# JinPLu/VeloxSeg

Measured on AMD Instinct MI355X. Metric: training patches/s on 128^3 2-mod volumes (fwd+loss+bwd+allreduce+AdamW), higher is better.
Workload: dtype f32

## Files before the change

include/veloxseg_hip.h:

```cpp
#ifndef VELOXSEG_HIP_H
#define VELOXSEG_HIP_H

#ifdef __cplusplus
extern "C" {
#endif

#define VX_ABI_VERSION 1

int vx_abi_version(void);
const char* vx_last_error(void);

int vx_conv3d_fwd(const float* x, const float* x2, int C1, const float* w, const float* bias, float* y,
                  int B, int Cin, int Di, int Hi, int Wi, int Cout, int K, int S, int P, int G, int ps, void* stream);
int vx_conv3d_bwd_data(const float* dy, const float* w, const float* bias_like, float* dx, float* dx2, int C1,
                       int B, int Cin, int Di, int Hi, int Wi, int Cout, int K, int S, int P, int G, int ps,
                       int accumulate, void* stream);
int vx_conv3d_bwd_weight(const float* x, const float* x2, int C1, const float* dy, float* dw, float* db,
                         int B, int Cin, int Di, int Hi, int Wi, int Cout, int K, int S, int P, int G, int ps, void* stream);

int vx_conv3d_bwd_weight_tiled(const float* x, const float* x2, int C1, const float* dy, float* dw, float* db,
                               int B, int Cin, int Di, int Hi, int Wi, int Cout, int K, int S, int P, int G, int ps, void* stream);
int vx_down_wgrad_ws_floats(int B, int Cin, int Di, int Hi, int Wi, int Cout);
int vx_down_wgrad_mfma(const float* x, const float* dy, float* dw, float* db, float* ws, long ws_floats,
                       int B, int Cin, int Di, int Hi, int Wi, int Cout, void* stream);
// ... 33 lines not shown
int vx_pw_conv_set_v4(int on);
int vx_pw_conv_bwd_data(const float* dy, const float* w, float* dx, float* dx2, int C1,
                        int B, int Cin, int Cout, long V, int accumulate, void* stream);
int vx_pw_conv_bwd_weight(const float* x, const float* x2, int C1, const float* dy, float* dw, float* db,
                          int B, int Cin, int Cout, long V, void* stream);
int vx_pw_conv_fwd_h(const void* x, const float* w, const float* bias, float* y, int B, int Cin, int Cout, long V, int x_h16, void* stream);
int vx_pw_conv_bwd_weight_h(const void* x, const float* dy, float* dw, float* db, int B, int Cin, int Cout, long V, int x_h16, void* stream);

int vx_pw_conv_mfma(const float* src, const float* src2, int S1, const float* w, int transpose_w, const float* bias,
                    float* dst, float* dst2, int D1, int B, int Mch, int Kch, int Cin_of_w, long V, int accumulate, void* stream);
int vx_pw_conv_bwd_fused(const float* dy, const float* w, const float* x, const float* x2, int C1, float* dx, float* dx2, float* dw, float* db,
                         int B, int Cin, int Cout, long V, int accumulate, void* stream);
int vx_pw_conv_bwd_fused_big(const float* dy, const float* w, const float* x, const float* x2, int C1, float* dx, float* dx2, float* dw, float* db,
                             int B, int Cin, int Cout, long V, int accumulate, void* stream);
int vx_pw_conv_gelu_fwd(const float* x, const float* w, const float* bias, float* a, float* h, int B, int Cin, int Cout, long V, int mfma,
                        const void* seed_ptr, unsigned long long dstream, float p, void* stream);
int vx_pw_conv_gelu_bwd_data(const float* dy, const float* w, const float* a, float* da, int B, int Cin, int Cout, long V, int mfma,
                             const void* seed_ptr, unsigned long long dstream, float p, void* stream);
int vx_pw_conv_res_fwd(const float* x, const float* w, const float* bias, const float* res, float* out, int B, int Cin, int Cout, long V, int mfma,
                       float alpha, const void* seed_ptr, unsigned long long dstream, float p, void* stream);
int vx_pw_mfma_set_wide(int on);

int vx_mlp_supported(int C, int R, long V);
int vx_mlp_bwd_nparts(int B, int C, long V);
int vx_mlp_fwd(const float* x, int norm, const double* part, int nparts, float* stats, const float* gamma, const float* beta,
               const float* w1, const float* b1, const float* w2, const float* b2, float* out, int B, int C, int R, long V, float eps,
               const void* seed_ptr, unsigned long long site1, float p1, unsigned long long site2, float p2, void* stream);
int vx_mlp_bwd(const float* x, int norm, const float* stats, const float* gamma, const float* beta, const float* w1, const float* b1,
               const float* w2, const float* dout, float* dx, float* part_out, float* dgamma, float* dbeta, float* dw1, float* db1,
               float* dw2, float* db2, int B, int C, int R, long V, float eps, const void* seed_ptr, unsigned long long site1, float p1,
               unsigned long long site2, float p2, void* stream);
int vx_jlc_ntiles(int B, int C, int G, int D, int H, int W);
int vx_jlc_nchunks(long BC, long V);
int vx_jlc_conv_fwd(const float* x, const float* w1, const float* w3, const float* w5, const float* b1, const float* b3, const float* b5,
                    float* y1, float* y3, float* y5, double* part, int B, int C, int G, int D, int H, int W, void* stream);
int vx_jlc_mid_fwd(const float* x, const float* y1, const float* y3, const float* y5, const double* part_y, int nty, float* stats_y, float* o,
                   double* part_o, long BC, long V, float eps, void* stream);
int vx_jlc_mid_bwd(const float* dout, const float* dn, const float* part_dn, int npd, const float* o, const float* stats_o, const float* y1,
                   const float* y3, const float* y5, const float* stats_y, float* d_o, float* part_t, long BC, long V, void* stream);
int vx_jlc_gk(const float* d_o, const float* y1, const float* y3, const float* y5, const float* stats_y, const float* part_t, float* g1, float* g3,
              float* g5, long BC, long V, void* stream);
int vx_jlc_conv_bwd(const float* g1, const float* g3, const float* g5, const float* w1, const float* w3, const float* w5, const float* d_o,
                    float* dx, int B, int C, int G, int D, int H, int W, void* stream);
int vx_jlc_mid_fwd_h(const float* x, const void* y1, const void* y3, const void* y5, const double* part_y, int nty, float* stats_y, void* o,
                     double* part_o, long BC, long V, float eps, int h16, void* stream);
int vx_jlc_mid_bwd_h(const float* dout, const void* dn, const float* part_dn, int npd, const void* o, const float* stats_o, const void* y1,
                     const void* y3, const void* y5, const float* stats_y, void* d_o, float* part_t, long BC, long V, int h16, void* stream);
int vx_jlc_gk_h(const void* d_o, const void* y1, const void* y3, const void* y5, const float* stats_y, const float* part_t, void* g1, void* g3,
                void* g5, long BC, long V, int h16, void* stream);
int vx_mlp_fwd_h(const void* x, int norm, const double* part, int nparts, float* stats, const float* gamma, const float* beta,
                 const float* w1, const float* b1, const float* w2, const float* b2, float* out, int B, int C, int R, long V, float eps,
                 const void* seed_ptr, unsigned long long site1, float p1, unsigned long long site2, float p2, int h16, void* stream);
int vx_mlp_bwd_h(const void* x, int norm, const float* stats, const float* gamma, const float* beta, const float* w1, const float* b1,
                 const float* w2, const float* dout, void* dx, float* part_out, float* dgamma, float* dbeta, float* dw1, float* db1,
                 float* dw2, float* db2, int B, int C, int R, long V, float eps, const void* seed_ptr, unsigned long long site1, float p1,
                 unsigned long long site2, float p2, int h16, void* stream);

int vx_jlc_tz_ok(int C, int G, int D, int H, int W);
int vx_jlc_tz_ntiles(int C, int G, int D, int H, int W);
int vx_jlc_tz_img_floats(int C, int G);
int vx_jlc_tz_set_pieces(int ns);
int vx_jlc_tz_set_min_voxels(long v);
int vx_jlc_tz_pieces(void);
int vx_jlc_tz_set_debug(int mask);
int vx_jlc_tz_prep(const float* w1, const float* w3, const float* w5, float* img, int C, int G, void* stream);
int vx_jlc_tz_fwd(const float* x, const float* img, const float* b1, const float* b3, const float* b5, float* y1, float* y3, float* y5, double* part,
                  int B, int C, int G, int D, int H, int W, void* stream);
int vx_jlc_tz_bwd(const float* g1, const float* g3, const float* g5, const float* img, const float* w1, const float* d_o, float* dx,
                  int B, int C, int G, int D, int H, int W, void* stream);
int vx_jlc_cl_ok(int C, int G, int D, int H, int W);
int vx_jlc_cl_ntiles(int C, int G, int D, int H, int W);
int vx_jlc_cl_img_floats(int C, int G);
int vx_jlc_cl_set_enabled(int on);
int vx_jlc_cl_prep(const float* w1, const float* w3, const float* w5, float* img, int C, int G, void* stream);
int vx_jlc_cl_fwd(const float* x, const float* img, const float* b1, const float* b3, const float* b5, float* y1, float* y3, float* y5, double* part,
                  int B, int C, int G, int D, int H, int W, void* stream);
int vx_jlc_cl_bwd(const float* g1, const float* g3, const float* g5, const float* img, const float* d_o, float* dx, int B, int C, int G, int D, int H, int W,
                  void* stream);
int vx_jlc_wgrad_tz_ok(int C, int G, int D, int H, int W);
int vx_jlc_wgrad_tz_set_min_voxels(long v);
int vx_jlc_wgrad_tz_set_blocks(int n);
int vx_jlc_wgrad_tz_set_spec(int on);
int vx_jlc_wgrad_tz_set_f16(int on);
int vx_jlc_wgrad_tz(const float* x, const float* g1, const float* g3, const float* g5, float* dw1, float* dw3, float* dw5, int B, int C, int G, int D, int H, int W,
                    void* stream);
int vx_jlc_tz_img_floats_ns(int C, int G, int pieces);
int vx_jlc_tz_prep_ns(const float* w1, const float* w3, const float* w5, float* img, int C, int G, int pieces, void* stream);
int vx_jlc_tz_fwd_ns(const float* x, const float* img, const float* b1, const float* b3, const float* b5, float* y1, float* y3, float* y5, double* part,
                     int B, int C, int G, int D, int H, int W, int pieces, void* stream);
int vx_jlc_tz_bwd_ns(const float* g1, const float* g3, const float* g5, const float* img, const float* w1, const float* d_o, float* dx,
                     int B, int C, int G, int D, int H, int W, int pieces, void* stream);
int vx_jlc_wgrad_tz_ns(const float* x, const float* g1, const float* g3, const float* g5, float* dw1, float* dw3, float* dw5, int B, int C, int G, int D, int H, int W,
                       int pieces, void* stream);
int vx_jlc_tz_fwd_h(const float* x, const float* img, const float* b1, const float* b3, const float* b5, void* y1, void* y3, void* y5, double* part,
// ... 246 lines not shown
```

veloxseg_amd/csrc/_vxops.cpp:

```cpp
#include <torch/extension.h>
#include <torch/csrc/autograd/custom_function.h>
#include <torch/custom_class.h>
#include <torch/library.h>
#include <c10/hip/HIPStream.h>
#include <ATen/hip/impl/HIPStreamMasqueradingAsCUDA.h>
#include <ATen/hip/impl/HIPGuardImplMasqueradingAsCUDA.h>
#include <hip/hip_runtime_api.h>
#include <algorithm>
#include <map>
#include <unordered_map>
#include <tuple>
#include <functional>
#include <type_traits>
#include <memory>
#include <vector>
#include <map>
#include <tuple>
#include "../../include/veloxseg_hip.h"

using at::Tensor;
typedef c10::optional<Tensor> OptT;

namespace {

// ... 990 lines not shown
            out = axpy_fwd_impl(st->r, o, z, 1.0, p, site, sp(rs), s_);
        }
        return {out, st};
    }

static Tensor jlc_bwd_f(std::shared_ptr<JLCState> st, const Tensor& dout_in, bool need_x, int64_t stream) {
        void* s_ = sp(stream);
        if (st->blk) {
            JLCFusedState& f = st->f;
            Tensor dout = contig(dout_in);
            const int B = f.B, C = f.C, G = f.G, D = f.D, H = f.H, W = f.W, R = f.R;
            const long V = (long)D * H * W, BC = (long)B * C, n1 = BC * V;
            const int npd = f.tile ? vx_inmlp_tiles(V) : vx_mlp_bwd_nparts(B, C, V);
            auto iopt = f.h16 ? f.x.options().dtype(at::kBFloat16) : f.x.options();
            const long esz = f.h16 ? 2 : 4;
            const int h16 = f.h16 ? 1 : 0;
            Tensor dn = at::empty(f.x.sizes(), iopt), part_dn = at::empty({BC, (long)npd, 2}, f.x.options());
            if (f.tile) {
                Tensor sc_n = at::empty_like(f.x), sc_dz = at::empty_like(f.x), sc_h = at::empty({B, R, D, H, W}, f.x.options()), sc_da = at::empty({B, R, D, H, W}, f.x.options());
                VX(vx_inmlp_bwd, fp(f.o), fp(f.stats_o), fp(f.l1w), fp(f.l1b), fp(f.l2w), fp(dout), mp(dn), mp(part_dn), mp(sc_n), mp(sc_h), mp(sc_da), mp(sc_dz), B, C, R, V,
                                 f.rs, (unsigned long long)f.site, (float)f.p, s_);
                float *dw1 = grad_ptr(f.l1w), *db1 = grad_ptr(f.l1b), *dw2 = grad_ptr(f.l2w), *db2 = grad_ptr(f.l2b);
                wgrad_submit(s_, f.x.device().index(), [=](void* s) {
                    const void* ptrs[8] = {fp(sc_h), fp(sc_dz), dw2, db2, fp(sc_n), fp(sc_da), dw1, db1};
                    const long dims[8] = {R, C, V, B, C, R, V, B};
                    VX(vx_pw_wgrad_group, ptrs, dims, 2, nullptr, nullptr, 0, s);
                });
            } else
            VX(vx_mlp_bwd_h, (const void*)f.o.data_ptr(), 0, fp(f.stats_o), nullptr, nullptr, fp(f.l1w), fp(f.l1b), fp(f.l2w), fp(dout), dn.data_ptr(), mp(part_dn), nullptr, nullptr,
                           grad_ptr(f.l1w), grad_ptr(f.l1b), grad_ptr(f.l2w), grad_ptr(f.l2b), B, C, R, V, (float)F.in_eps, f.rs, 0ull, 0.0f,
                           (unsigned long long)f.site, (float)f.p, h16, s_);
            const char* yp = (const char*)f.y.data_ptr();
            const void *y1 = yp, *y3 = yp + esz * n1, *y5 = yp + 2 * esz * n1;
            Tensor d_o = at::empty(f.x.sizes(), iopt), part_t = at::empty({3, BC, (long)f.nch, 2}, f.x.options());
            VX(vx_jlc_mid_bwd_h, fp(dout), (const void*)dn.data_ptr(), fp(part_dn), npd, (const void*)f.o.data_ptr(), fp(f.stats_o), y1, y3, y5, fp(f.stats_y), d_o.data_ptr(), mp(part_t), BC, V, h16, s_);
            Tensor g = at::empty({3, B, C, D, H, W}, iopt);
            char* gp = (char*)g.data_ptr();
            void *g1 = gp, *g3 = gp + esz * n1, *g5 = gp + 2 * esz * n1;
            VX(vx_jlc_gk_h, (const void*)d_o.data_ptr(), y1, y3, y5, fp(f.stats_y), fp(part_t), g1, g3, g5, BC, V, h16, s_);
            Tensor dx;
            if (need_x) {
                dx = f.h16 ? at::empty_like(f.x) : dn;
                if (f.img.defined() && f.img_cl) VX(vx_jlc_cl_bwd, (const float*)g1, (const float*)g3, (const float*)g5, fp(f.img), fp(d_o), mp(dx), B, C, G, D, H, W, s_);
                else if (f.img.defined()) VX(vx_jlc_tz_bwd_h, (const void*)g1, (const void*)g3, (const void*)g5, fp(f.img), fp(f.w1), (const void*)d_o.data_ptr(), mp(dx), B, C, G, D, H, W, f.tz_pieces, h16, s_);
                else
                VX(vx_jlc_conv_bwd, (const float*)g1, (const float*)g3, (const float*)g5, fp(f.w1), fp(f.w3), fp(f.w5), fp(d_o), mp(dx), B, C, G, D, H, W, s_);
            }
            grad_ptr(f.b1); grad_ptr(f.b3); grad_ptr(f.b5);
            const int Cg = C / G;
            {
                Tensor xk = f.x, gk = g;
                float* dw1 = f.w1.requires_grad() ? grad_ptr(f.w1) : nullptr;
                float* dw3 = f.w3.requires_grad() ? grad_ptr(f.w3) : nullptr;
                float* dw5 = f.w5.requires_grad() ? grad_ptr(f.w5) : nullptr;
                const bool g1fast = F.use_gconv1 && (Cg == 4 || Cg == 8 || Cg == 16) && V % 4 == 0;
                const bool tzok = F.jlc_wg_tz && dw1 && dw3 && dw5 && vx_jlc_wgrad_tz_ok(C, G, D, H, W);
                const bool wga = F.jlc_wg_tz && dw1 && dw3 && dw5 && vx_jlc_wgrad_gather_ok(C, G, D, H, W) == 1 && (!tzok || V <= 64);
                const bool wtz = !wga && tzok;
                const int wg_pieces = f.tz_pieces ? f.tz_pieces : vx_jlc_tz_pieces();
                wgrad_submit(s_, f.x.device().index(), [=](void* s) {
                    if (h16) {
                        const char* gh = (const char*)gk.data_ptr();
                        TORCH_CHECK(wtz, "veloxseg_amd.jlc: the 16-bit g_k of the bf16 storage mode need the matrix-pipe weight-gradient kernel");
                        VX(vx_jlc_wgrad_tz_h, fp(xk), (const void*)gh, (const void*)(gh + 2 * n1), (const void*)(gh + 4 * n1), dw1, dw3, dw5, B, C, G, D, H, W, wg_pieces, 1, s);
                        return;
                    }
                    const float* gq = gk.data_ptr<float>();
                    if (wga) {
                        VX(vx_jlc_wgrad_gather, fp(xk), gq, gq + n1, gq + 2 * n1, dw1, dw3, dw5, B, C, G, D, H, W, s);
                        return;
                    }
                    if (wtz) {
// ... 642 lines not shown
```

veloxseg_amd/csrc/jlc.hip:

```cpp
#include "vx_common.h"
#include "../../include/veloxseg_hip.h"

struct VxJlc {
    const float *x, *w1, *w3, *w5, *b1, *b3, *b5;
    const float *g1, *g3, *g5, *res;
    float *y1, *y3, *y5, *dx;
    double* part;
    int B, C, G, D, H, W;
    int TD, TH, TWq, nTd, nTh, nTw, cic, nthr;
    int parts, nsp;
};

template <int K>
__device__ __forceinline__ void vx_jlc_stage(const float* __restrict__ src, float* __restrict__ xs, const VxJlc& p, int b, int c_first, int ncc,
                                             int d0, int h0, int w0, int HD, int HH, int HWp) {
    constexpr int P = K / 2;
    const int tid = threadIdx.x, nthr = p.nthr;
    int hw = tid % HWp, t1 = tid / HWp;
    int hh = t1 % HH, t2 = t1 / HH;
    int hd = t2 % HD, cil = t2 / HD;
    int r = nthr;
    const int st_hw = r % HWp; r /= HWp;
    const int st_hh = r % HH; r /= HH;
    const int st_hd = r % HD; r /= HD;
// ... 361 lines not shown
            st[2 * k] = mean; st[2 * k + 1] = rstd;
            if (blockIdx.x == 0) { p.stats_y_out[((long)k * p.BC + bc) * 2] = mean; p.stats_y_out[((long)k * p.BC + bc) * 2 + 1] = rstd; }
        }
    }
    __syncthreads();
    const float m1 = st[0], r1 = st[1], m3 = st[2], r3 = st[3], m5 = st[4], r5 = st[5];
    const long base = bc * p.V, c0 = (long)blockIdx.x * p.chunk;
    const long c1 = c0 + p.chunk < p.V ? c0 + p.chunk : p.V;
    float s = 0.0f, q = 0.0f;
    for (long i = c0 + 4 * tid; i < c1; i += 1024) {
        const float4 xv = vx_ld4(p.x, base + i), a = vx_ld4(y1, base + i), b3 = vx_ld4(y3, base + i), c5 = vx_ld4(y5, base + i);
        float4 o;
        o.x = xv.x + vx_gelu_fast((a.x - m1) * r1) + vx_gelu_fast((b3.x - m3) * r3) + vx_gelu_fast((c5.x - m5) * r5);
        o.y = xv.y + vx_gelu_fast((a.y - m1) * r1) + vx_gelu_fast((b3.y - m3) * r3) + vx_gelu_fast((c5.y - m5) * r5);
        o.z = xv.z + vx_gelu_fast((a.z - m1) * r1) + vx_gelu_fast((b3.z - m3) * r3) + vx_gelu_fast((c5.z - m5) * r5);
        o.w = xv.w + vx_gelu_fast((a.w - m1) * r1) + vx_gelu_fast((b3.w - m3) * r3) + vx_gelu_fast((c5.w - m5) * r5);
        o.x = vx_round_as<TI>(o.x); o.y = vx_round_as<TI>(o.y); o.z = vx_round_as<TI>(o.z); o.w = vx_round_as<TI>(o.w);
        vx_st4(out_o, base + i, o);
        s += (o.x + o.y) + (o.z + o.w);
        q = fmaf(o.x, o.x, q); q = fmaf(o.y, o.y, q); q = fmaf(o.z, o.z, q); q = fmaf(o.w, o.w, q);
    }
    s = vx_wave_sum(s);
    q = vx_wave_sum(q);
    if ((tid & 63) == 0) { redd[2 * (tid >> 6)] = (double)s; redd[2 * (tid >> 6) + 1] = (double)q; }
    __syncthreads();
    if (tid == 0) {
        double* dst = p.part_o + (bc * p.nch + blockIdx.x) * 2;
        dst[0] = (redd[0] + redd[2]) + (redd[4] + redd[6]);
        dst[1] = (redd[1] + redd[3]) + (redd[5] + redd[7]);
    }
}

template <typename TI>
__global__ void __launch_bounds__(256) vx_jlc_mid_bwd_k(VxJlcMid p) {
    const TI* __restrict__ y1 = (const TI*)p.y1; const TI* __restrict__ y3 = (const TI*)p.y3; const TI* __restrict__ y5 = (const TI*)p.y5;
    const TI* __restrict__ o_ = (const TI*)p.o; const TI* __restrict__ dn_ = (const TI*)p.dn;
    TI* __restrict__ out_do = (TI*)p.out_do;
    __shared__ float mm[2];
    __shared__ float redf[4][6];
    const long bc = blockIdx.y;
    const int tid = threadIdx.x;
    if (tid < 64) {
        float s, q;
        vx_fold_f(p.part_dn + bc * p.npd * 2, p.npd, s, q);
        if (tid == 0) { mm[0] = s / (float)p.V; mm[1] = q / (float)p.V; }
    }
    __syncthreads();
    const float dm1 = mm[0], dm2 = mm[1];
    const float mo = p.stats_o[2 * bc], ro = p.stats_o[2 * bc + 1];
    float mk[3], rk[3];
#pragma unroll
    for (int k = 0; k < 3; ++k) { mk[k] = p.stats_y[((long)k * p.BC + bc) * 2]; rk[k] = p.stats_y[((long)k * p.BC + bc) * 2 + 1]; }
    const long base = bc * p.V, c0 = (long)blockIdx.x * p.chunk;
    const long c1 = c0 + p.chunk < p.V ? c0 + p.chunk : p.V;
    float acc[6] = {0.f, 0.f, 0.f, 0.f, 0.f, 0.f};
    for (long i = c0 + 4 * tid; i < c1; i += 1024) {
        const float4 go = vx_ld4(p.dout, base + i), dn = vx_ld4(dn_, base + i), ov = vx_ld4(o_, base + i);
        const float4 a = vx_ld4(y1, base + i), b3 = vx_ld4(y3, base + i), c5 = vx_ld4(y5, base + i);
        const float gov[4] = {go.x, go.y, go.z, go.w}, dnv[4] = {dn.x, dn.y, dn.z, dn.w}, oo[4] = {ov.x, ov.y, ov.z, ov.w};
        const float yv[3][4] = {{a.x, a.y, a.z, a.w}, {b3.x, b3.y, b3.z, b3.w}, {c5.x, c5.y, c5.z, c5.w}};
        float dv[4];
#pragma unroll
        for (int u = 0; u < 4; ++u) {
            const float nh = (oo[u] - mo) * ro;
            dv[u] = vx_round_as<TI>(gov[u] + ro * (dnv[u] - dm1 - nh * dm2));
#pragma unroll
            for (int k = 0; k < 3; ++k) {
                const float yh = (yv[k][u] - mk[k]) * rk[k];
                const float t = dv[u] * vx_gelu_grad_fast(yh);
                acc[2 * k] += t;
                acc[2 * k + 1] = fmaf(t, yh, acc[2 * k + 1]);
            }
        }
        vx_st4(out_do, base + i, make_float4(dv[0], dv[1], dv[2], dv[3]));
    }
#pragma unroll
    for (int e = 0; e < 6; ++e) {
        const float t = vx_wave_sum(acc[e]);
        if ((tid & 63) == 0) redf[tid >> 6][e] = t;
    }
    __syncthreads();
    if (tid < 6) {
        const int k = tid >> 1;
        p.part_t[(((long)k * p.BC + bc) * p.nch + blockIdx.x) * 2 + (tid & 1)] = (redf[0][tid] + redf[1][tid]) + (redf[2][tid] + redf[3][tid]);
    }
}

template <typename TI>
__global__ void __launch_bounds__(256) vx_jlc_gk_k(VxJlcMid p) {
    const TI* __restrict__ y1 = (const TI*)p.y1; const TI* __restrict__ y3 = (const TI*)p.y3; const TI* __restrict__ y5 = (const TI*)p.y5;
    const TI* __restrict__ d_o = (const TI*)p.d_o;
    TI* __restrict__ g1 = (TI*)p.g1; TI* __restrict__ g3 = (TI*)p.g3; TI* __restrict__ g5 = (TI*)p.g5;
    __shared__ float mm[6];
    const long bc = blockIdx.y;
    const int tid = threadIdx.x;
    if (tid < 192) {
        const int k = tid >> 6;
        float s, q;
        vx_fold_f(p.part_t_in + ((long)k * p.BC + bc) * p.nch * 2, p.nch, s, q);
        if ((tid & 63) == 0) { mm[2 * k] = s / (float)p.V; mm[2 * k + 1] = q / (float)p.V; }
    }
    __syncthreads();
    float mk[3], rk[3], t1[3], t2[3];
#pragma unroll
    for (int k = 0; k < 3; ++k) {
        mk[k] = p.stats_y[((long)k * p.BC + bc) * 2]; rk[k] = p.stats_y[((long)k * p.BC + bc) * 2 + 1];
        t1[k] = mm[2 * k]; t2[k] = mm[2 * k + 1];
    }
    const long base = bc * p.V, c0 = (long)blockIdx.x * p.chunk;
    const long c1 = c0 + p.chunk < p.V ? c0 + p.chunk : p.V;
    for (long i = c0 + 4 * tid; i < c1; i += 1024) {
        const float4 dv = vx_ld4(d_o, base + i);
        const float4 a = vx_ld4(y1, base + i), b3 = vx_ld4(y3, base + i), c5 = vx_ld4(y5, base + i);
        const float d4[4] = {dv.x, dv.y, dv.z, dv.w};
        const float yv[3][4] = {{a.x, a.y, a.z, a.w}, {b3.x, b3.y, b3.z, b3.w}, {c5.x, c5.y, c5.z, c5.w}};
        float gk[3][4];
#pragma unroll
        for (int k = 0; k < 3; ++k)
#pragma unroll
            for (int u = 0; u < 4; ++u) {
                const float yh = (yv[k][u] - mk[k]) * rk[k];
                const float t = d4[u] * vx_gelu_grad_fast(yh);
                gk[k][u] = rk[k] * (t - t1[k] - yh * t2[k]);
            }
        vx_st4(g1, base + i, make_float4(gk[0][0], gk[0][1], gk[0][2], gk[0][3]));
        vx_st4(g3, base + i, make_float4(gk[1][0], gk[1][1], gk[1][2], gk[1][3]));
        vx_st4(g5, base + i, make_float4(gk[2][0], gk[2][1], gk[2][2], gk[2][3]));
    }
}

static int vx_jlc_geom(VxJlc& p, int B, int C, int G, int D, int H, int W, int K, int& COT, size_t& shm) {
    VX_REQUIRE(B > 0 && C > 0 && G > 0 && C % G == 0 && D > 0 && H > 0 && W > 0, "vx_jlc: bad shape");
    const int Cg = C / G;
    VX_REQUIRE(Cg % 4 == 0, "vx_jlc: group width must be a multiple of 4 (got %d)", Cg);
    p.B = B; p.C = C; p.G = G; p.D = D; p.H = H; p.W = W;
    p.TWq = vx_cdiv(W, 4) < 8 ? vx_cdiv(W, 4) : 8;
    p.TH = H < 8 ? H : 8;
    int td = 256 / (p.TWq * p.TH);
    if (td > D) td = D;
    if (td > 8) td = 8;
    if (td < 1) td = 1;
    p.TD = td;
    auto nblk = [&]() { return (long)vx_cdiv(D, p.TD) * vx_cdiv(H, p.TH) * vx_cdiv(W, p.TWq * 4) * (C / COT) * 4; };
    COT = 4;
    while (p.TD > 1 && nblk() < 128 && (p.TD / 2) * p.TWq * p.TH >= 64) p.TD /= 2;
    p.nTd = vx_cdiv(D, p.TD); p.nTh = vx_cdiv(H, p.TH); p.nTw = vx_cdiv(W, p.TWq * 4);
    p.nsp = (p.TD * p.TH * p.TWq + 63) / 64 * 64;
    if (p.nsp > 256) p.nsp = 256;
    const int plane = (p.TD + K - 1) * (p.TH + K - 1) * (p.TWq * 4 + 4);
    const int taps = K == 5 ? 153 : 125;
    int cic = Cg < 4 ? Cg : 4;
    auto lds = [&](int c) { return (size_t)c * (plane + taps * COT) * sizeof(float); };
    while (cic > 1 && lds(cic) > 64 * 1024) cic >>= 1;
    p.parts = 1;
    if (nblk() < 512) {
        if (cic % 4 == 0 && p.nsp * 4 <= 512 && nblk() < 384) p.parts = 4;
        else if (cic % 2 == 0 && p.nsp * 2 <= 512) p.parts = 2;
    }
    p.nthr = p.nsp * p.parts;
    p.cic = cic;
// ... 12 lines not shown

extern "C" int vx_jlc_conv_fwd(const float* x, const float* w1, const float* w3, const float* w5, const float* b1, const float* b3, const float* b5,
                               float* y1, float* y3, float* y5, double* part, int B, int C, int G, int D, int H, int W, void* stream) {
    VX_REQUIRE(x && w1 && w3 && w5 && y1 && y3 && y5 && part, "vx_jlc_conv_fwd: null pointer");
    VxJlc p = {};
    int COT; size_t shm;
    if (int rc = vx_jlc_geom(p, B, C, G, D, H, W, 5, COT, shm)) return rc;
    p.x = x; p.w1 = w1; p.w3 = w3; p.w5 = w5; p.b1 = b1; p.b3 = b3; p.b5 = b5; p.y1 = y1; p.y3 = y3; p.y5 = y5; p.part = part;
    dim3 grid(p.nTd * p.nTh * p.nTw, C / COT, B);
    hipStream_t st = (hipStream_t)stream;
    if (COT == 4) vx_jlc_conv_fwd_k<4><<<grid, dim3(p.nthr), shm, st>>>(p);
    else if (COT == 2) vx_jlc_conv_fwd_k<2><<<grid, dim3(p.nthr), shm, st>>>(p);
    else vx_jlc_conv_fwd_k<1><<<grid, dim3(p.nthr), shm, st>>>(p);
    VX_LAUNCH_CHECK("vx_jlc_conv_fwd");
    return 0;
}

extern "C" int vx_jlc_conv_bwd(const float* g1, const float* g3, const float* g5, const float* w1, const float* w3, const float* w5, const float* d_o,
                               float* dx, int B, int C, int G, int D, int H, int W, void* stream) {
    VX_REQUIRE(g1 && g3 && g5 && w1 && w3 && w5 && d_o && dx, "vx_jlc_conv_bwd: null pointer");
    VxJlc p = {};
    int COT; size_t shm;
    if (int rc = vx_jlc_geom(p, B, C, G, D, H, W, 5, COT, shm)) return rc;
    p.g1 = g1; p.g3 = g3; p.g5 = g5; p.w1 = w1; p.w3 = w3; p.w5 = w5; p.res = d_o; p.dx = dx;
    dim3 grid(p.nTd * p.nTh * p.nTw, C / COT, B);
    hipStream_t st = (hipStream_t)stream;
    if (COT == 4) vx_jlc_conv_bwd_k<4><<<grid, dim3(p.nthr), shm, st>>>(p);
    else if (COT == 2) vx_jlc_conv_bwd_k<2><<<grid, dim3(p.nthr), shm, st>>>(p);
    else vx_jlc_conv_bwd_k<1><<<grid, dim3(p.nthr), shm, st>>>(p);
    VX_LAUNCH_CHECK("vx_jlc_conv_bwd");
    return 0;
}

static long vx_jlc_chunk(long BC, long V) {
    (void)BC;
    return V >= 16384 ? 4096 : 1024;
}
extern "C" int vx_jlc_nchunks(long BC, long V) { return vx_cdiv(V, vx_jlc_chunk(BC, V)); }

extern "C" int vx_jlc_mid_fwd_h(const float* x, const void* y1, const void* y3, const void* y5, const double* part_y, int nty, float* stats_y, void* o,
                                double* part_o, long BC, long V, float eps, int h16, void* stream) {
    VX_REQUIRE(x && y1 && y3 && y5 && part_y && stats_y && o && part_o && BC > 0 && V > 0 && V % 4 == 0, "vx_jlc_mid_fwd: bad args");
    VxJlcMid p = {};
    p.x = x; p.y1 = y1; p.y3 = y3; p.y5 = y5; p.part_y = part_y; p.nty = nty; p.stats_y_out = stats_y; p.out_o = o; p.part_o = part_o;
    p.BC = BC; p.V = V; p.eps = eps; p.chunk = vx_jlc_chunk(BC, V); p.nch = vx_cdiv(V, p.chunk);
    if (h16) vx_jlc_mid_fwd_k<vx_bf16><<<dim3(p.nch, (unsigned)BC), dim3(256), 0, (hipStream_t)stream>>>(p);
    else vx_jlc_mid_fwd_k<float><<<dim3(p.nch, (unsigned)BC), dim3(256), 0, (hipStream_t)stream>>>(p);
    VX_LAUNCH_CHECK("vx_jlc_mid_fwd");
    return 0;
}
extern "C" int vx_jlc_mid_fwd(const float* x, const float* y1, const float* y3, const float* y5, const double* part_y, int nty, float* stats_y, float* o,
                              double* part_o, long BC, long V, float eps, void* stream) {
    return vx_jlc_mid_fwd_h(x, y1, y3, y5, part_y, nty, stats_y, o, part_o, BC, V, eps, 0, stream);
}

extern "C" int vx_jlc_mid_bwd_h(const float* dout, const void* dn, const float* part_dn, int npd, const void* o, const float* stats_o, const void* y1,
                                const void* y3, const void* y5, const float* stats_y, void* d_o, float* part_t, long BC, long V, int h16, void* stream) {
    VX_REQUIRE(dout && dn && part_dn && o && stats_o && y1 && y3 && y5 && stats_y && d_o && part_t && BC > 0 && V > 0 && V % 4 == 0, "vx_jlc_mid_bwd: bad args");
    VxJlcMid p = {};
    p.dout = dout; p.dn = dn; p.part_dn = part_dn; p.npd = npd; p.o = o; p.stats_o = stats_o; p.y1 = y1; p.y3 = y3; p.y5 = y5; p.stats_y = stats_y;
    p.out_do = d_o; p.part_t = part_t; p.BC = BC; p.V = V; p.chunk = vx_jlc_chunk(BC, V); p.nch = vx_cdiv(V, p.chunk);
    if (h16) vx_jlc_mid_bwd_k<vx_bf16><<<dim3(p.nch, (unsigned)BC), dim3(256), 0, (hipStream_t)stream>>>(p);
    else vx_jlc_mid_bwd_k<float><<<dim3(p.nch, (unsigned)BC), dim3(256), 0, (hipStream_t)stream>>>(p);
    VX_LAUNCH_CHECK("vx_jlc_mid_bwd");
    return 0;
}
extern "C" int vx_jlc_mid_bwd(const float* dout, const float* dn, const float* part_dn, int npd, const float* o, const float* stats_o, const float* y1,
                              const float* y3, const float* y5, const float* stats_y, float* d_o, float* part_t, long BC, long V, void* stream) {
    return vx_jlc_mid_bwd_h(dout, dn, part_dn, npd, o, stats_o, y1, y3, y5, stats_y, d_o, part_t, BC, V, 0, stream);
}

extern "C" int vx_jlc_gk_h(const void* d_o, const void* y1, const void* y3, const void* y5, const float* stats_y, const float* part_t, void* g1, void* g3,
                           void* g5, long BC, long V, int h16, void* stream) {
    VX_REQUIRE(d_o && y1 && y3 && y5 && stats_y && part_t && g1 && g3 && g5 && BC > 0 && V > 0 && V % 4 == 0, "vx_jlc_gk: bad args");
    VxJlcMid p = {};
    p.d_o = d_o; p.y1 = y1; p.y3 = y3; p.y5 = y5; p.stats_y = stats_y; p.part_t_in = part_t; p.g1 = g1; p.g3 = g3; p.g5 = g5;
    p.BC = BC; p.V = V; p.chunk = vx_jlc_chunk(BC, V); p.nch = vx_cdiv(V, p.chunk);
    if (h16) vx_jlc_gk_k<vx_bf16><<<dim3(p.nch, (unsigned)BC), dim3(256), 0, (hipStream_t)stream>>>(p);
    else vx_jlc_gk_k<float><<<dim3(p.nch, (unsigned)BC), dim3(256), 0, (hipStream_t)stream>>>(p);
    VX_LAUNCH_CHECK("vx_jlc_gk");
    return 0;
}
extern "C" int vx_jlc_gk(const float* d_o, const float* y1, const float* y3, const float* y5, const float* stats_y, const float* part_t, float* g1, float* g3,
                         float* g5, long BC, long V, void* stream) {
    return vx_jlc_gk_h(d_o, y1, y3, y5, stats_y, part_t, g1, g3, g5, BC, V, 0, stream);
}
```

veloxseg_amd/csrc/jlc_mfma.hip:

```cpp
#include "vx_common.h"
#include <type_traits>
#include "../../include/veloxseg_hip.h"

typedef __bf16 tz_bf8 __attribute__((ext_vector_type(8)));
typedef float tz_f4 __attribute__((ext_vector_type(4)));

struct TzGeo {
    int HD, HH;
    int Sd, Sc, Sp;
    int nrows;
    unsigned mHH, mHD;
    int qd0, nq;
    unsigned mNQ;
};

struct VxTz {
    const void* src[3];
    const uint4* img;
    const float* esc;
    const float* bias[3];
    const void* res;
    const float* w1;
    void* out[3];
    double* part;
// ... 522 lines not shown
static unsigned tz_magic(int d) { return d <= 1 ? 0u : (unsigned)(((1ull << 32) + d - 1) / (unsigned long long)d); }

static int g_tz_pieces = 22;
static thread_local int t_tz_pieces = 0;
static inline int tz_pieces() { return t_tz_pieces ? t_tz_pieces : g_tz_pieces; }
namespace { struct TzPiecesScope { int prev; explicit TzPiecesScope(int ns) : prev(t_tz_pieces) { t_tz_pieces = ns; } ~TzPiecesScope() { t_tz_pieces = prev; } }; }
static inline bool tz_pieces_valid(int ns) { return (ns >= 1 && ns <= 3) || ns == 22; }
static thread_local int t_tz_h16 = 0;
namespace { struct TzH16Scope { int prev; explicit TzH16Scope(int h) : prev(t_tz_h16) { t_tz_h16 = h; } ~TzH16Scope() { t_tz_h16 = prev; } }; }
static int g_tz_dbg = 0;
extern "C" int vx_jlc_tz_set_debug(int mask) { g_tz_dbg = mask; return 0; }
extern "C" int vx_jlc_tz_set_pieces(int ns) { if (!((ns >= 1 && ns <= 3) || ns == 22)) return -1; g_tz_pieces = ns; return 0; }
static inline int tz_ns(int pieces) { return pieces == 22 ? 2 : pieces; }
extern "C" int vx_jlc_tz_pieces(void) { return g_tz_pieces; }

struct TzPlan { int CG, NT, MTW, nwaves; size_t shm; };

static void tz_geo(TzGeo& ge, const VxTz& p, int CG, int hw) {
    ge.HD = p.TD + 2 * hw; ge.HH = p.TH + 2 * hw;
    ge.Sd = ge.HH * p.RW;
    if (p.TWB >= 2) {
        const int iv = 4 * p.TWB;
        while (!((ge.Sd % iv) == 0 && ((ge.Sd / iv) & 1) && true)) ge.Sd += 4;
    }
    ge.Sc = ge.HD * ge.Sd;
    while ((ge.Sc & 127) != 64) ge.Sc += 4;
    ge.Sp = CG * ge.Sc;
    ge.nrows = CG * ge.HD * ge.HH;
    ge.mHH = tz_magic(ge.HH); ge.mHD = tz_magic(ge.HD);
    if (hw == 0) { ge.qd0 = 1; ge.nq = p.TWB; } else { ge.qd0 = 0; ge.nq = p.TWB + 2; }
    ge.mNQ = tz_magic(ge.nq);
}

static int tz_plan(VxTz& p, TzPlan& pl, int B, int C, int G, int D, int H, int W, int pieces) {
    const int NS = tz_ns(pieces);
    if (B <= 0 || C <= 0 || G <= 0 || C % G || D <= 0 || H <= 0 || W <= 0 || (W & 3)) return -1;
    const int CG = C / G;
    if (CG != 4 && CG != 8 && CG != 16) return -1;
    p.B = B; p.C = C; p.G = G; p.D = D; p.H = H; p.W = W;
    constexpr int tdm = 8, thm = 8;
    p.TWB = W / 4 < 8 ? W / 4 : 8;
    p.TH = H < thm ? H : thm;
    p.TD = D < tdm ? D : tdm;
    auto lds_bytes = [&](int td, int th, int twb) {
        VxTz q = p; TzGeo ge;
        q.TD = td; q.TH = th; q.TWB = twb; q.RW = 4 * twb + 4;
        tz_geo(ge, q, CG, 2);
        return (size_t)NS * ge.Sp * 2;
    };
    while (lds_bytes(p.TD, p.TH, p.TWB) > 150 * 1024) {
        if (p.TD > 1 && p.TD >= p.TH) p.TD = (p.TD + 1) / 2;
        else if (p.TH > 1) p.TH = (p.TH + 1) / 2;
        else return -1;
    }
    p.nTd = vx_cdiv(D, p.TD); p.nTh = vx_cdiv(H, p.TH); p.nTw = vx_cdiv(W / 4, p.TWB);
    p.RW = 4 * p.TWB + 4;
    p.P = p.TD * p.TH * p.TWB;
    p.nNt = vx_cdiv(p.P, 16);
    p.mTWB = tz_magic(p.TWB); p.mTD = tz_magic(p.TD);
    tz_geo(p.geo[0], p, CG, 2);
    tz_geo(p.geo[1], p, CG, 1);
    const int MT = CG / 4;
    pl.CG = CG;
    int best = -1;
    pl.NT = 1; pl.MTW = 1;
    for (int mtw = 1; mtw <= MT; mtw <<= 1)
        for (int nt = 1; nt <= 4; nt <<= 1) {
            if (mtw * nt > 4) continue;
            const int waves = (MT / mtw) * vx_cdiv(p.nNt, nt);
            if (waves > 8) continue;
            const int score = waves * 100 + mtw * 10 + nt;
            if (score > best) { best = score; pl.NT = nt; pl.MTW = mtw; }
        }
    if (best < 0) return -1;
    pl.nwaves = (MT / pl.MTW) * vx_cdiv(p.nNt, pl.NT);
    if (pl.nwaves > 8) return -1;
    if (pieces == 22) {
        const long nthr = 64L * pl.nwaves;
        if ((long)p.geo[0].nrows * p.geo[0].nq > TZ_NQ16 * nthr || (long)p.geo[1].nrows * p.geo[1].nq > TZ_NQ16 * nthr) return -1;
    }
    size_t halo = lds_bytes(p.TD, p.TH, p.TWB);
    halo = (halo + 15) & ~(size_t)15;
    p.red_off = (int)halo;
    pl.shm = halo + (size_t)3 * pl.nwaves * pl.MTW * 4 * 2 * sizeof(float);
    return 0;
}

static long g_tz_min_v = 1024;
extern "C" int vx_jlc_tz_set_min_voxels(long v) { g_tz_min_v = v < 0 ? 0 : v; return 0; }
extern "C" int vx_jlc_tz_ok(int C, int G, int D, int H, int W) {
    VxTz p = {};
    TzPlan pl;
    if ((long)D * H * W < g_tz_min_v) return 0;
    return tz_plan(p, pl, 1, C, G, D, H, W, tz_pieces()) == 0 ? 1 : 0;
}
extern "C" int vx_jlc_tz_ntiles(int C, int G, int D, int H, int W) {
    VxTz p = {};
    TzPlan pl;
    if (tz_plan(p, pl, 1, C, G, D, H, W, tz_pieces()) != 0) return -1;
    return p.nTd * p.nTh * p.nTw;
}
static long tz_img_elems(int C, int G, int pieces) {
    const int NS = tz_ns(pieces);
    const int CG = C / G, MT = CG / 4;
    return (long)G * 35 * MT * MT * NS * 64 + (long)2 * MT * MT * NS * 64;
}
extern "C" int vx_jlc_tz_img_floats(int C, int G) { return (int)(2 * tz_img_elems(C, G, tz_pieces()) * 4 + ((3 * G + 3) & ~3)); }

extern "C" int vx_jlc_tz_prep(const float* w1, const float* w3, const float* w5, float* img, int C, int G, void* stream) {
    VX_REQUIRE(w1 && w3 && w5 && img && G > 0 && C % G == 0, "vx_jlc_tz_prep: bad args");
    const int CG = C / G, NS = tz_ns(tz_pieces());
    VX_REQUIRE(CG == 4 || CG == 8 || CG == 16, "vx_jlc_tz_prep: group width %d", CG);
    const long ne = tz_img_elems(C, G, tz_pieces());
    uint4* f = reinterpret_cast<uint4*>(img);
// ... 613 lines not shown
```

Measured before the change: 1083.

## Fuse JLC mid-bwd and gk kernels for small volumes; shrink tz tiles for occupancy

For rows with V ≤ 4096, a new single-kernel path launches one block per (b,c) row. That kernel computes d_o, reduces the GELU-gradient partials in shared memory, and writes g1/g3/g5 straight from registers. This removes the second kernel launch, the part_t round trip, and the re-reading of d_o and y1/y3/y5. Separately, the tz conv planner halves TD/TH until at least 256 blocks exist, except when CG is 16, which trades more halo overhead for occupancy. It also adds tunable hooks for the long-chunk size and the block target, and switches the arithmetic to explicit fmaf with contraction off.

```diff
diff --git a/include/veloxseg_hip.h b/include/veloxseg_hip.h
--- a/include/veloxseg_hip.h
+++ b/include/veloxseg_hip.h
@@ -89,6 +89,7 @@
                unsigned long long site2, float p2, void* stream);
 int vx_jlc_ntiles(int B, int C, int G, int D, int H, int W);
 int vx_jlc_nchunks(long BC, long V);
+int vx_jlc_set_long_chunk(long n);
 int vx_jlc_conv_fwd(const float* x, const float* w1, const float* w3, const float* w5, const float* b1, const float* b3, const float* b5,
                     float* y1, float* y3, float* y5, double* part, int B, int C, int G, int D, int H, int W, void* stream);
 int vx_jlc_mid_fwd(const float* x, const float* y1, const float* y3, const float* y5, const double* part_y, int nty, float* stats_y, float* o,
@@ -99,12 +100,18 @@
               float* g5, long BC, long V, void* stream);
 int vx_jlc_conv_bwd(const float* g1, const float* g3, const float* g5, const float* w1, const float* w3, const float* w5, const float* d_o,
                     float* dx, int B, int C, int G, int D, int H, int W, void* stream);
+int vx_jlc_mid_bwd_gk_ok(long BC, long V);
+int vx_jlc_mid_bwd_gk(const float* dout, const float* dn, const float* part_dn, int npd, const float* o, const float* stats_o, const float* y1,
+                      const float* y3, const float* y5, const float* stats_y, float* d_o, float* g1, float* g3, float* g5, long BC, long V, void* stream);
 int vx_jlc_mid_fwd_h(const float* x, const void* y1, const void* y3, const void* y5, const double* part_y, int nty, float* stats_y, void* o,
                      double* part_o, long BC, long V, float eps, int h16, void* stream);
 int vx_jlc_mid_bwd_h(const float* dout, const void* dn, const float* part_dn, int npd, const void* o, const float* stats_o, const void* y1,
                      const void* y3, const void* y5, const float* stats_y, void* d_o, float* part_t, long BC, long V, int h16, void* stream);
 int vx_jlc_gk_h(const void* d_o, const void* y1, const void* y3, const void* y5, const float* stats_y, const float* part_t, void* g1, void* g3,
                 void* g5, long BC, long V, int h16, void* stream);
+int vx_jlc_mid_bwd_gk_h(const float* dout, const void* dn, const float* part_dn, int npd, const void* o, const float* stats_o, const void* y1,
+                        const void* y3, const void* y5, const float* stats_y, void* d_o, void* g1, void* g3, void* g5, long BC, long V, int h16,
+                        void* stream);
 int vx_mlp_fwd_h(const void* x, int norm, const double* part, int nparts, float* stats, const float* gamma, const float* beta,
                  const float* w1, const float* b1, const float* w2, const float* b2, float* out, int B, int C, int R, long V, float eps,
                  const void* seed_ptr, unsigned long long site1, float p1, unsigned long long site2, float p2, int h16, void* stream);
@@ -117,6 +124,7 @@
 int vx_jlc_tz_ntiles(int C, int G, int D, int H, int W);
 int vx_jlc_tz_img_floats(int C, int G);
 int vx_jlc_tz_set_pieces(int ns);
+int vx_jlc_tz_set_block_target(int n);
 int vx_jlc_tz_set_min_voxels(long v);
 int vx_jlc_tz_pieces(void);
 int vx_jlc_tz_set_debug(int mask);
diff --git a/veloxseg_amd/csrc/_vxops.cpp b/veloxseg_amd/csrc/_vxops.cpp
--- a/veloxseg_amd/csrc/_vxops.cpp
+++ b/veloxseg_amd/csrc/_vxops.cpp
@@ -1046,12 +1046,17 @@
                            (unsigned long long)f.site, (float)f.p, h16, s_);
             const char* yp = (const char*)f.y.data_ptr();
             const void *y1 = yp, *y3 = yp + esz * n1, *y5 = yp + 2 * esz * n1;
-            Tensor d_o = at::empty(f.x.sizes(), iopt), part_t = at::empty({3, BC, (long)f.nch, 2}, f.x.options());
-            VX(vx_jlc_mid_bwd_h, fp(dout), (const void*)dn.data_ptr(), fp(part_dn), npd, (const void*)f.o.data_ptr(), fp(f.stats_o), y1, y3, y5, fp(f.stats_y), d_o.data_ptr(), mp(part_t), BC, V, h16, s_);
+            Tensor d_o = at::empty(f.x.sizes(), iopt);
             Tensor g = at::empty({3, B, C, D, H, W}, iopt);
             char* gp = (char*)g.data_ptr();
             void *g1 = gp, *g3 = gp + esz * n1, *g5 = gp + 2 * esz * n1;
-            VX(vx_jlc_gk_h, (const void*)d_o.data_ptr(), y1, y3, y5, fp(f.stats_y), fp(part_t), g1, g3, g5, BC, V, h16, s_);
+            if (vx_jlc_mid_bwd_gk_ok(BC, V)) {
+                VX(vx_jlc_mid_bwd_gk_h, fp(dout), (const void*)dn.data_ptr(), fp(part_dn), npd, (const void*)f.o.data_ptr(), fp(f.stats_o), y1, y3, y5, fp(f.stats_y), d_o.data_ptr(), g1, g3, g5, BC, V, h16, s_);
+            } else {
+                Tensor part_t = at::empty({3, BC, (long)vx_jlc_nchunks(BC, V), 2}, f.x.options());
+                VX(vx_jlc_mid_bwd_h, fp(dout), (const void*)dn.data_ptr(), fp(part_dn), npd, (const void*)f.o.data_ptr(), fp(f.stats_o), y1, y3, y5, fp(f.stats_y), d_o.data_ptr(), mp(part_t), BC, V, h16, s_);
+                VX(vx_jlc_gk_h, (const void*)d_o.data_ptr(), y1, y3, y5, fp(f.stats_y), fp(part_t), g1, g3, g5, BC, V, h16, s_);
+            }
             Tensor dx;
             if (need_x) {
                 dx = f.h16 ? at::empty_like(f.x) : dn;
diff --git a/veloxseg_amd/csrc/jlc.hip b/veloxseg_amd/csrc/jlc.hip
--- a/veloxseg_amd/csrc/jlc.hip
+++ b/veloxseg_amd/csrc/jlc.hip
@@ -417,10 +417,59 @@
 }
 
 template <typename TI>
+__device__ __forceinline__ float vx_jlc_do_elem(float go, float dn, float o, float mo, float ro, float dm1, float dm2) {
+#pragma clang fp contract(off)
+    const float nh = (o - mo) * ro;
+    return vx_round_as<TI>(fmaf(ro, fmaf(-nh, dm2, dn - dm1), go));
+}
+__device__ __forceinline__ float vx_jlc_t_elem(float d, float y, float mk, float rk, float& yh) {
+#pragma clang fp contract(off)
+    yh = (y - mk) * rk;
+    return d * vx_gelu_grad_fast(yh);
+}
+__device__ __forceinline__ float vx_jlc_gk_elem(float d, float y, float mk, float rk, float t1, float t2) {
+#pragma clang fp contract(off)
+    const float yh = (y - mk) * rk;
+    return rk * fmaf(-yh, t2, fmaf(d, vx_gelu_grad_fast(yh), -t1));
+}
+template <typename TI>
+__device__ __forceinline__ void vx_jlc_mid_bwd_quad(const VxJlcMid& p, long off, float mo, float ro, float dm1, float dm2, const float (&mk)[3], const float (&rk)[3],
+                                                    float (&dv)[4], float (&yv)[3][4], float (&acc)[6]) {
+#pragma clang fp contract(off)
+    const float4 go = vx_ld4(p.dout, off), dn = vx_ld4((const TI*)p.dn, off), ov = vx_ld4((const TI*)p.o, off);
+    const float4 a = vx_ld4((const TI*)p.y1, off), b3 = vx_ld4((const TI*)p.y3, off), c5 = vx_ld4((const TI*)p.y5, off);
+    const float gov[4] = {go.x, go.y, go.z, go.w}, dnv[4] = {dn.x, dn.y, dn.z, dn.w}, oo[4] = {ov.x, ov.y, ov.z, ov.w};
+    yv[0][0] = a.x; yv[0][1] = a.y; yv[0][2] = a.z; yv[0][3] = a.w;
+    yv[1][0] = b3.x; yv[1][1] = b3.y; yv[1][2] = b3.z; yv[1][3] = b3.w;
+    yv[2][0] = c5.x; yv[2][1] = c5.y; yv[2][2] = c5.z; yv[2][3] = c5.w;
+#pragma unroll
+    for (int u = 0; u < 4; ++u) {
+        dv[u] = vx_jlc_do_elem<TI>(gov[u], dnv[u], oo[u], mo, ro, dm1, dm2);
+#pragma unroll
+        for (int k = 0; k < 3; ++k) {
+            float yh;
+            const float t = vx_jlc_t_elem(dv[u], yv[k][u], mk[k], rk[k], yh);
+            acc[2 * k] += t;
+            acc[2 * k + 1] = fmaf(t, yh, acc[2 * k + 1]);
+        }
+    }
+    vx_st4((TI*)p.out_do, off, make_float4(dv[0], dv[1], dv[2], dv[3]));
+}
+template <typename TI>
+__device__ __forceinline__ void vx_jlc_gk_quad(const VxJlcMid& p, long off, const float (&d4)[4], const float (&yv)[3][4], const float (&mk)[3], const float (&rk)[3],
+                                               const float (&t1)[3], const float (&t2)[3]) {
+    float gk[3][4];
+#pragma unroll
+    for (int k = 0; k < 3; ++k)
+#pragma unroll
+        for (int u = 0; u < 4; ++u) gk[k][u] = vx_jlc_gk_elem(d4[u], yv[k][u], mk[k], rk[k], t1[k], t2[k]);
+    vx_st4((TI*)p.g1, off, make_float4(gk[0][0], gk[0][1], gk[0][2], gk[0][3]));
+    vx_st4((TI*)p.g3, off, make_float4(gk[1][0], gk[1][1], gk[1][2], gk[1][3]));
+    vx_st4((TI*)p.g5, off, make_float4(gk[2][0], gk[2][1], gk[2][2], gk[2][3]));
+}
+
+template <typename TI>
 __global__ void __launch_bounds__(256) vx_jlc_mid_bwd_k(VxJlcMid p) {
-    const TI* __restrict__ y1 = (const TI*)p.y1; const TI* __restrict__ y3 = (const TI*)p.y3; const TI* __restrict__ y5 = (const TI*)p.y5;
-    const TI* __restrict__ o_ = (const TI*)p.o; const TI* __restrict__ dn_ = (const TI*)p.dn;
-    TI* __restrict__ out_do = (TI*)p.out_do;
     __shared__ float mm[2];
     __shared__ float redf[4][6];
     const long bc = blockIdx.y;
@@ -440,24 +489,8 @@
     const long c1 = c0 + p.chunk < p.V ? c0 + p.chunk : p.V;
     float acc[6] = {0.f, 0.f, 0.f, 0.f, 0.f, 0.f};
     for (long i = c0 + 4 * tid; i < c1; i += 1024) {
-        const float4 go = vx_ld4(p.dout, base + i), dn = vx_ld4(dn_, base + i), ov = vx_ld4(o_, base + i);
-        const float4 a = vx_ld4(y1, base + i), b3 = vx_ld4(y3, base + i), c5 = vx_ld4(y5, base + i);
-        const float gov[4] = {go.x, go.y, go.z, go.w}, dnv[4] = {dn.x, dn.y, dn.z, dn.w}, oo[4] = {ov.x, ov.y, ov.z, ov.w};
-        const float yv[3][4] = {{a.x, a.y, a.z, a.w}, {b3.x, b3.y, b3.z, b3.w}, {c5.x, c5.y, c5.z, c5.w}};
-        float dv[4];
-#pragma unroll
-        for (int u = 0; u < 4; ++u) {
-            const float nh = (oo[u] - mo) * ro;
-            dv[u] = vx_round_as<TI>(gov[u] + ro * (dnv[u] - dm1 - nh * dm2));
-#pragma unroll
-            for (int k = 0; k < 3; ++k) {
-                const float yh = (yv[k][u] - mk[k]) * rk[k];
-                const float t = dv[u] * vx_gelu_grad_fast(yh);
-                acc[2 * k] += t;
-                acc[2 * k + 1] = fmaf(t, yh, acc[2 * k + 1]);
-            }
-        }
-        vx_st4(out_do, base + i, make_float4(dv[0], dv[1], dv[2], dv[3]));
+        float dv[4], yv[3][4];
+        vx_jlc_mid_bwd_quad<TI>(p, base + i, mo, ro, dm1, dm2, mk, rk, dv, yv, acc);
     }
 #pragma unroll
     for (int e = 0; e < 6; ++e) {
@@ -475,7 +508,6 @@
 __global__ void __launch_bounds__(256) vx_jlc_gk_k(VxJlcMid p) {
     const TI* __restrict__ y1 = (const TI*)p.y1; const TI* __restrict__ y3 = (const TI*)p.y3; const TI* __restrict__ y5 = (const TI*)p.y5;
     const TI* __restrict__ d_o = (const TI*)p.d_o;
-    TI* __restrict__ g1 = (TI*)p.g1; TI* __restrict__ g3 = (TI*)p.g3; TI* __restrict__ g5 = (TI*)p.g5;
     __shared__ float mm[6];
     const long bc = blockIdx.y;
     const int tid = threadIdx.x;
@@ -499,18 +531,56 @@
         const float4 a = vx_ld4(y1, base + i), b3 = vx_ld4(y3, base + i), c5 = vx_ld4(y5, base + i);
         const float d4[4] = {dv.x, dv.y, dv.z, dv.w};
         const float yv[3][4] = {{a.x, a.y, a.z, a.w}, {b3.x, b3.y, b3.z, b3.w}, {c5.x, c5.y, c5.z, c5.w}};
-        float gk[3][4];
-#pragma unroll
-        for (int k = 0; k < 3; ++k)
-#pragma unroll
-            for (int u = 0; u < 4; ++u) {
-                const float yh = (yv[k][u] - mk[k]) * rk[k];
-                const float t = d4[u] * vx_gelu_grad_fast(yh);
-                gk[k][u] = rk[k] * (t - t1[k] - yh * t2[k]);
-            }
-        vx_st4(g1, base + i, make_float4(gk[0][0], gk[0][1], gk[0][2], gk[0][3]));
-        vx_st4(g3, base + i, make_float4(gk[1][0], gk[1][1], gk[1][2], gk[1][3]));
-        vx_st4(g5, base + i, make_float4(gk[2][0], gk[2][1], gk[2][2], gk[2][3]));
+        vx_jlc_gk_quad<TI>(p, base + i, d4, yv, mk, rk, t1, t2);
+    }
+}
+
+template <typename TI>
+__global__ void __launch_bounds__(1024) vx_jlc_mid_bwd_gk_k(VxJlcMid p) {
+    __shared__ float mm[2];
+    __shared__ float redf[16][6];
+    __shared__ float pt[3][4][2];
+    __shared__ float mt[6];
+    const long bc = blockIdx.x;
+    const int tid = threadIdx.x;
+    if (tid < 64) {
+        float s, q;
+        vx_fold_f(p.part_dn + bc * p.npd * 2, p.npd, s, q);
+        if (tid == 0) { mm[0] = s / (float)p.V; mm[1] = q / (float)p.V; }
+    }
+    __syncthreads();
+    const float dm1 = mm[0], dm2 = mm[1];
+    const float mo = p.stats_o[2 * bc], ro = p.stats_o[2 * bc + 1];
+    float mk[3], rk[3];
+#pragma unroll
+    for (int k = 0; k < 3; ++k) { mk[k] = p.stats_y[((long)k * p.BC + bc) * 2]; rk[k] = p.stats_y[((long)k * p.BC + bc) * 2 + 1]; }
+    const long i = 4L * tid;
+    const bool live = i < p.V;
+    const long off = bc * p.V + i;
+    float acc[6] = {0.f, 0.f, 0.f, 0.f, 0.f, 0.f};
+    float dv[4] = {0.f, 0.f, 0.f, 0.f}, yv[3][4] = {};
+    if (live) vx_jlc_mid_bwd_quad<TI>(p, off, mo, ro, dm1, dm2, mk, rk, dv, yv, acc);
+#pragma unroll
+    for (int e = 0; e < 6; ++e) {
+        const float t = vx_wave_sum(acc[e]);
+        if ((tid & 63) == 0) redf[tid >> 6][e] = t;
+    }
+    __syncthreads();
+    if (tid < 6 * p.nch) {
+        const int j = tid / 6, e = tid - 6 * j;
+        pt[e >> 1][j][e & 1] = (redf[4 * j][e] + redf[4 * j + 1][e]) + (redf[4 * j + 2][e] + redf[4 * j + 3][e]);
+    }
+    __syncthreads();
+    if (tid < 192) {
+        const int k = tid >> 6;
+        float s, q;
+        vx_fold_f(&pt[k][0][0], p.nch, s, q);
+        if ((tid & 63) == 0) { mt[2 * k] = s / (float)p.V; mt[2 * k + 1] = q / (float)p.V; }
+    }
+    __syncthreads();
+    if (live) {
+        const float t1[3] = {mt[0], mt[2], mt[4]}, t2[3] = {mt[1], mt[3], mt[5]};
+        vx_jlc_gk_quad<TI>(p, off, dv, yv, mk, rk, t1, t2);
     }
 }
 
@@ -589,9 +659,15 @@
     return 0;
 }
 
+static long g_jlc_long_chunk = 0;
+extern "C" int vx_jlc_set_long_chunk(long n) {
+    if (n != 0 && (n < 1024 || n > 8192 || n % 1024)) return -1;
+    g_jlc_long_chunk = n;
+    return 0;
+}
 static long vx_jlc_chunk(long BC, long V) {
     (void)BC;
-    return V >= 16384 ? 4096 : 1024;
+    return V >= 16384 ? (g_jlc_long_chunk ? g_jlc_long_chunk : 4096) : 1024;
 }
 extern "C" int vx_jlc_nchunks(long BC, long V) { return vx_cdiv(V, vx_jlc_chunk(BC, V)); }
 
@@ -642,3 +718,24 @@
                          float* g5, long BC, long V, void* stream) {
     return vx_jlc_gk_h(d_o, y1, y3, y5, stats_y, part_t, g1, g3, g5, BC, V, 0, stream);
 }
+
+extern "C" int vx_jlc_mid_bwd_gk_ok(long BC, long V) { return BC > 0 && V > 0 && V % 4 == 0 && V <= 4096 ? 1 : 0; }
+
+extern "C" int vx_jlc_mid_bwd_gk_h(const float* dout, const void* dn, const float* part_dn, int npd, const void* o, const float* stats_o, const void* y1,
+                                   const void* y3, const void* y5, const float* stats_y, void* d_o, void* g1, void* g3, void* g5, long BC, long V, int h16,
+                                   void* stream) {
+    VX_REQUIRE(dout && dn && part_dn && o && stats_o && y1 && y3 && y5 && stats_y && d_o && g1 && g3 && g5, "vx_jlc_mid_bwd_gk: null pointer");
+    VX_REQUIRE(vx_jlc_mid_bwd_gk_ok(BC, V) == 1, "vx_jlc_mid_bwd_gk: one block per row needs V %% 4 == 0 and V <= 4096 (got BC = %ld, V = %ld)", BC, V);
+    VxJlcMid p = {};
+    p.dout = dout; p.dn = dn; p.part_dn = part_dn; p.npd = npd; p.o = o; p.stats_o = stats_o; p.y1 = y1; p.y3 = y3; p.y5 = y5; p.stats_y = stats_y;
+    p.out_do = d_o; p.g1 = g1; p.g3 = g3; p.g5 = g5; p.BC = BC; p.V = V; p.chunk = vx_jlc_chunk(BC, V); p.nch = vx_cdiv(V, p.chunk);
+    VX_REQUIRE(p.chunk == 1024 && p.nch >= 1 && p.nch <= 4, "vx_jlc_mid_bwd_gk: chunk %ld x %d", p.chunk, p.nch);
+    if (h16) vx_jlc_mid_bwd_gk_k<vx_bf16><<<dim3((unsigned)BC), dim3(256 * p.nch), 0, (hipStream_t)stream>>>(p);
+    else vx_jlc_mid_bwd_gk_k<float><<<dim3((unsigned)BC), dim3(256 * p.nch), 0, (hipStream_t)stream>>>(p);
+    VX_LAUNCH_CHECK("vx_jlc_mid_bwd_gk");
+    return 0;
+}
+extern "C" int vx_jlc_mid_bwd_gk(const float* dout, const float* dn, const float* part_dn, int npd, const float* o, const float* stats_o, const float* y1,
+                                 const float* y3, const float* y5, const float* stats_y, float* d_o, float* g1, float* g3, float* g5, long BC, long V, void* stream) {
+    return vx_jlc_mid_bwd_gk_h(dout, dn, part_dn, npd, o, stats_o, y1, y3, y5, stats_y, d_o, g1, g3, g5, BC, V, 0, stream);
+}
diff --git a/veloxseg_amd/csrc/jlc_mfma.hip b/veloxseg_amd/csrc/jlc_mfma.hip
--- a/veloxseg_amd/csrc/jlc_mfma.hip
+++ b/veloxseg_amd/csrc/jlc_mfma.hip
@@ -578,6 +578,16 @@
     ge.mNQ = tz_magic(ge.nq);
 }
 
+static int g_tz_block_target = 0;
+extern "C" int vx_jlc_tz_set_block_target(int n) { g_tz_block_target = n > 0 ? n : 0; return 0; }
+static long tz_block_target(int CG, int G, int D, int H, int W) {
+    (void)G; (void)D; (void)H; (void)W;
+    if (CG == 16) return 0;
+    if (g_tz_block_target > 0) return g_tz_block_target;
+    return 256;
+}
+
+static int tz_plan_tiles(VxTz& p, TzPlan& pl, int CG, int NS, int pieces, size_t halo);
 static int tz_plan(VxTz& p, TzPlan& pl, int B, int C, int G, int D, int H, int W, int pieces) {
     const int NS = tz_ns(pieces);
     if (B <= 0 || C <= 0 || G <= 0 || C % G || D <= 0 || H <= 0 || W <= 0 || (W & 3)) return -1;
@@ -599,6 +609,26 @@
         else if (p.TH > 1) p.TH = (p.TH + 1) / 2;
         else return -1;
     }
+    if (tz_plan_tiles(p, pl, CG, NS, pieces, lds_bytes(p.TD, p.TH, p.TWB)) != 0) return -1;
+    int td = p.TD, th = p.TH;
+    const long target = tz_block_target(CG, G, D, H, W);
+    auto nblk = [&]() { return 4L * G * vx_cdiv(D, td) * vx_cdiv(H, th) * vx_cdiv(W / 4, p.TWB); };
+    while (nblk() < target) {
+        int& t = td >= th ? td : th;
+        if (t / 2 < 4) break;
+        t = (t + 1) / 2;
+    }
+    if (td != p.TD || th != p.TH) {
+        VxTz q = p;
+        TzPlan ql;
+        q.TD = td; q.TH = th;
+        if (tz_plan_tiles(q, ql, CG, NS, pieces, lds_bytes(td, th, p.TWB)) == 0) { p = q; pl = ql; }
+    }
+    return 0;
+}
+
+static int tz_plan_tiles(VxTz& p, TzPlan& pl, int CG, int NS, int pieces, size_t halo) {
+    const int D = p.D, H = p.H, W = p.W;
     p.nTd = vx_cdiv(D, p.TD); p.nTh = vx_cdiv(H, p.TH); p.nTw = vx_cdiv(W / 4, p.TWB);
     p.RW = 4 * p.TWB + 4;
     p.P = p.TD * p.TH * p.TWB;
@@ -625,7 +655,6 @@
         const long nthr = 64L * pl.nwaves;
         if ((long)p.geo[0].nrows * p.geo[0].nq > TZ_NQ16 * nthr || (long)p.geo[1].nrows * p.geo[1].nq > TZ_NQ16 * nthr) return -1;
     }
-    size_t halo = lds_bytes(p.TD, p.TH, p.TWB);
     halo = (halo + 15) & ~(size_t)15;
     p.red_off = (int)halo;
     pl.shm = halo + (size_t)3 * pl.nwaves * pl.MTW * 4 * 2 * sizeof(float);
```

After: 1090, median of 6. About the same (+0.6%).
